# csteinmetz1/st-ito

Measured on AMD Instinct MI355X. Metric: candidate-evals/sec (pop x iters), 48 kHz 10 s stereo, 5-effect chain, higher is better.
Workload: dtype f32 (effects f32 / f64 as the reference; trunk convs with >= 256 output channels: f32 operands carried as f16 hi + lo pairs on the f16 matrix pipe, f32 accumulate -- as close to float64 as the f32 pipe, tools/ubench/split_mfma.hip)

## Files before the change

### st-ito_amd/csrc/compressor.hip

```cpp
#include "common.h"
#include "dsp_view.h"
#include "comp_scan.inc"

namespace stito {

static constexpr int CB_K = 15;
static constexpr int CB_TILE = 128;
static constexpr int CB_D = STITO_COMP_SCAN_DEPTH;
static constexpr int CA_TILE = 256;
static constexpr float CB_CMIN = 1.0e-30f;

typedef float cb_f2 __attribute__((ext_vector_type(2)));
typedef float cb_f4 __attribute__((ext_vector_type(4)));

struct CompGeom {
    int64_t L;
    int64_t n_blocks;
    int64_t n_fn;
    int64_t fn_stride;
    int64_t z_stride;
};

static CompGeom comp_geometry(int64_t L) {
    CompGeom g;
    g.L = L;
    g.n_blocks = (L + CB_K - 1) / CB_K;
    g.n_fn = g.n_blocks - 1;
    g.fn_stride = (g.n_fn + 2 * CB_D) * 16;
    g.z_stride = (g.n_fn + CB_D - 1) / CB_D * CB_D + CB_D;
    return g;
}

struct CompLayout : WsLayout { size_t fn, z_end; };
static CompLayout comp_layout(int n_streams, const CompGeom &g) {
    CompLayout l;
    l.fn = l.add((size_t)n_streams * g.fn_stride * sizeof(float));
    l.z_end = l.add((size_t)n_streams * g.z_stride * sizeof(float));
    return l;
}
size_t compressor_workspace_bytes(int n_streams, int64_t n_samples) { return comp_layout(n_streams, comp_geometry(n_samples)).total; }

struct CompCoef {
    float thr, thr_inv, p, cat, crl, sg;
};
__device__ __forceinline__ CompCoef comp_coef(const double *coef, int cand) {
    const double *cf = coef + (int64_t)cand * COEF_STRIDE;
    CompCoef c;
    c.thr = (float)cf[0];
    c.thr_inv = (float)cf[1];
    c.p = (float)cf[2];
    c.cat = (float)cf[3];
    c.crl = (float)cf[4];
    c.sg = c.cat <= c.crl ? 1.0f : -1.0f;
    return c;
}

template <int CTRL>
__device__ __forceinline__ float dpp(float old, float v) {
    return __builtin_bit_cast(float, __builtin_amdgcn_update_dpp(__builtin_bit_cast(int, old), __builtin_bit_cast(int, v),
                                                                 CTRL, 0xf, 0xf, false));
}

__global__ __launch_bounds__(256) void k_comp_blockfn(InView in, float *__restrict__ fn, CompGeom g, int C,
                                                       const double *__restrict__ coef) {
    __shared__ cb_f2 pairs[CB_TILE * CB_K];
    const int s = blockIdx.y, cand = s / C, ch = s % C;
    const float *x = in_ptr(in, cand, ch);
    const CompCoef cc = comp_coef(coef, cand);
    const float sa = cc.sg * (1.0f - cc.cat), sr = cc.sg * (1.0f - cc.crl);
    const cb_f2 c2 = {fmaxf(cc.cat, CB_CMIN), fmaxf(cc.crl, CB_CMIN)};
    const int64_t blk0 = (int64_t)blockIdx.x * CB_TILE, t0 = blk0 * CB_K;
    for (int i = threadIdx.x; i < CB_TILE * CB_K; i += 256) {
        const float v = t0 + i < g.L ? fabsf(x[t0 + i]) : 0.0f;
        pairs[i] = (cb_f2){sa * v, sr * v};
    }
    __syncthreads();
    const int lane = threadIdx.x & 63, w = threadIdx.x >> 6, row = lane >> 4, j = lane & 15;
    const float ninf = -__builtin_inff();
    float *out = fn + (int64_t)s * g.fn_stride;
#pragma unroll 2
    for (int it = 0; it < CB_TILE / 16; ++it) {
        const int bl = w * (CB_TILE / 4) + it * 4 + row;
        const cb_f2 *pr = pairs + bl * CB_K;
        float B = j == 0 ? 0.0f : ninf;
#pragma unroll
        for (int n = 0; n < CB_K; ++n) {
            const float sh = dpp<0x111>(ninf, B);
            const cb_f2 t = __builtin_elementwise_fma(c2, (cb_f2){sh, B}, pr[n]);
            B = fmaxf(t.x, t.y);
        }
        if (blk0 + bl < g.n_fn) out[(blk0 + bl) * 16 + j] = B;
    }
}

__global__ __launch_bounds__(64) void k_comp_blockscan(const float *__restrict__ fn, float *__restrict__ z_end, CompGeom g,
                                                        int C, int S, const double *__restrict__ coef, int spw) {
    const int lane = threadIdx.x, q = lane & 3;
    const int s_raw = blockIdx.x * spw + ((lane >> 2) & (spw - 1));
    const int s = s_raw < S ? s_raw : S - 1;
    const CompCoef cc = comp_coef(coef, s / C);
    const double ca = fmaxf(cc.cat, CB_CMIN), cr = fmaxf(cc.crl, CB_CMIN);
    float S4[4];
#pragma unroll
    for (int u = 0; u < 4; ++u) {
        const int jj = 4 * q + u;
        S4[u] = (float)(pow(ca, (double)jj) * pow(cr, (double)(CB_K - jj)));
    }
    const cb_f2 S01 = {S4[0], S4[1]}, S23 = {S4[2], S4[3]};
    const cb_f4 *src = (const cb_f4 *)(fn + (int64_t)s * g.fn_stride) + q;
    float *dst = z_end + (int64_t)s * g.z_stride;
    const int64_t n_ring = (g.n_fn + CB_D - 1) / CB_D;
    STITO_COMP_SCAN_PROLOGUE(src, dst + n_ring * CB_D);
    float z = 0.0f;
    for (int64_t r = 0; r < n_ring; ++r) {
        STITO_COMP_SCAN_PASS(z, S01, S23, src, dst);
        src += 4 * CB_D;
        dst += CB_D;
    }
    STITO_COMP_SCAN_DRAIN();
}

__device__ __forceinline__ float vca_gain(float e, float thr, float thr_inv, float p) {
    return e < thr ? 1.0f : __builtin_amdgcn_exp2f(p * __builtin_amdgcn_logf(e * thr_inv));
}

__global__ __launch_bounds__(CA_TILE) void k_comp_apply(InView in, float *out, const float *__restrict__ z_end,
                                                         CompGeom g, int64_t cand_stride, int C,
                                                         const double *__restrict__ coef) {
    __shared__ float tile[CA_TILE * CB_K];
    const int s = blockIdx.y, cand = s / C, ch = s % C;
    const float *x = in_ptr(in, cand, ch);
    float *y = out + (int64_t)cand * cand_stride + (int64_t)ch * g.L;
    const CompCoef cc = comp_coef(coef, cand);
    const int64_t blk0 = (int64_t)blockIdx.x * CA_TILE, t0 = blk0 * CB_K;
    const int n_here = (int)((g.L - t0 < CA_TILE * CB_K) ? g.L - t0 : CA_TILE * CB_K);
    for (int i = threadIdx.x; i < n_here; i += CA_TILE) tile[i] = x[t0 + i];
    const int64_t k = blk0 + threadIdx.x;
    float env = (k > 0 && k < g.n_blocks) ? fabsf(z_end[(int64_t)s * g.z_stride + k - 1]) : 0.0f;
    __syncthreads();
    float *mine = tile + threadIdx.x * CB_K;
    if (threadIdx.x * CB_K < n_here) {
#pragma unroll
        for (int n = 0; n < CB_K; ++n) {
            const float xv = mine[n], v = fabsf(xv);
            const float c = v > env ? cc.cat : cc.crl;
            env = __fadd_rn(v, __fmul_rn(c, __fsub_rn(env, v)));
            mine[n] = vca_gain(env, cc.thr, cc.thr_inv, cc.p) * xv;
        }
    }
    __syncthreads();
    for (int i = threadIdx.x; i < n_here; i += CA_TILE) y[t0 + i] = tile[i];
}

int compressor_stage(const InView &in, float *audio_dev, int64_t cand_stride, int pop, int C, int64_t n_samples,
                     const double *coef, void *workspace, hipStream_t st) {
    const CompGeom g = comp_geometry(n_samples);
    const int S = pop * C;
    const CompLayout l = comp_layout(S, g);
    float *fn = (float *)((char *)workspace + l.fn), *z_end = (float *)((char *)workspace + l.z_end);
    if (g.n_fn > 0) {
        hipLaunchKernelGGL(k_comp_blockfn, dim3((unsigned)((g.n_fn + CB_TILE - 1) / CB_TILE), S), dim3(256), 0, st, in, fn, g, C, coef);
        STITO_LAUNCH_CHECK();
        DeviceInfo dinfo;
        STITO_TRY(device_info(dinfo));
        int spw = 8;
        while (spw > 1 && (S + spw - 1) / spw < dinfo.cus / 4) spw >>= 1;
        if (const char *e = getenv("STITO_COMP_SPW")) { const int v = atoi(e); if (v >= 1 && v <= 16 && (v & (v - 1)) == 0) spw = v; }
        hipLaunchKernelGGL(k_comp_blockscan, dim3((S + spw - 1) / spw), dim3(64), 0, st, fn, z_end, g, C, S, coef, spw);
        STITO_LAUNCH_CHECK();
    }
    hipLaunchKernelGGL(k_comp_apply, dim3((unsigned)((g.n_blocks + CA_TILE - 1) / CA_TILE), S), dim3(CA_TILE), 0, st, in, audio_dev,
                       z_end, g, cand_stride, C, coef);
    STITO_LAUNCH_CHECK();
    return STITO_OK;
}

}
```

Measured before the change: 6048.

## Fuse compressor blockfn, scan and apply into one warp-specialized persistent kernel

Adds a single fused kernel per stream (or stream pair) in which producer waves compute block max-plus functions into LDS, one wave runs the serial scan in hand-written assembly, and consumer waves apply the gain and write output. The segments are pipelined across steps with double/triple-buffered LDS and barriers. This removes the global round-trips of the fn and z_end workspaces and two kernel launches. In exchange, parallelism is limited to one workgroup per stream or stream pair, and the code relies on hard-coded registers in inline asm. It becomes the default path and can be disabled with an environment variable.

Measured after the change: 6169 (median of 6 runs). 2.0% higher.

```diff
diff --git a/st-ito_amd/csrc/comp_stage.inc b/st-ito_amd/csrc/comp_stage.inc
--- /dev/null
+++ b/st-ito_amd/csrc/comp_stage.inc
@@ -0,0 +1,774 @@
+#define STITO_COMP_STAGE_G 64
+#define STITO_COMP_STAGE_SEGMENT(z, s01, s23, fn_lds, z_lds) \
+    asm volatile( \
+        "ds_write_b32 %4, %0 offset:12\n\t" \
+        "ds_read_b128 v[40:43], %3 offset:0\n\t" \
+        "ds_read_b128 v[44:47], %3 offset:64\n\t" \
+        "ds_read_b128 v[48:51], %3 offset:128\n\t" \
+        "ds_read_b128 v[52:55], %3 offset:192\n\t" \
+        "ds_read_b128 v[56:59], %3 offset:256\n\t" \
+        "ds_read_b128 v[60:63], %3 offset:320\n\t" \
+        "ds_read_b128 v[64:67], %3 offset:384\n\t" \
+        "ds_read_b128 v[68:71], %3 offset:448\n\t" \
+        "s_waitcnt lgkmcnt(4)\n\t" \
+        "v_mov_b32 v84, %0\n\t" \
+        "v_pk_fma_f32 v[80:81], %1, v[84:85], v[40:41] op_sel_hi:[1,0,1]\n\t" \
+        "v_pk_fma_f32 v[82:83], %2, v[84:85], v[42:43] op_sel_hi:[1,0,1]\n\t" \
+        "v_max_f32 v84, v80, v81\n\t" \
+        "v_max3_f32 v84, v84, v82, v83\n\t" \
+        "ds_read_b128 v[40:43], %3 offset:512\n\t" \
+        "s_nop 0\n\t" \
+        "v_max_f32_dpp v85, v84, v84 quad_perm:[1,0,3,2] row_mask:0xf bank_mask:0xf\n\t" \
+        "s_nop 1\n\t" \
+        "v_max_f32_dpp v72, v85, v85 quad_perm:[2,3,0,1] row_mask:0xf bank_mask:0xf\n\t" \
+        "v_pk_fma_f32 v[80:81], %1, v[72:73], v[44:45] op_sel_hi:[1,0,1]\n\t" \
+        "v_pk_fma_f32 v[82:83], %2, v[72:73], v[46:47] op_sel_hi:[1,0,1]\n\t" \
+        "v_max_f32 v84, v80, v81\n\t" \
+        "v_max3_f32 v84, v84, v82, v83\n\t" \
+        "ds_read_b128 v[44:47], %3 offset:576\n\t" \
+        "s_nop 0\n\t" \
+        "v_max_f32_dpp v85, v84, v84 quad_perm:[1,0,3,2] row_mask:0xf bank_mask:0xf\n\t" \
+        "s_nop 1\n\t" \
+        "v_max_f32_dpp v73, v85, v85 quad_perm:[2,3,0,1] row_mask:0xf bank_mask:0xf\n\t" \
+        "v_pk_fma_f32 v[80:81], %1, v[72:73], v[48:49] op_sel:[0,1,0] op_sel_hi:[1,1,1]\n\t" \
+        "v_pk_fma_f32 v[82:83], %2, v[72:73], v[50:51] op_sel:[0,1,0] op_sel_hi:[1,1,1]\n\t" \
+        "v_max_f32 v84, v80, v81\n\t" \
+        "v_max3_f32 v84, v84, v82, v83\n\t" \
+        "ds_read_b128 v[48:51], %3 offset:640\n\t" \
+        "s_nop 0\n\t" \
+        "v_max_f32_dpp v85, v84, v84 quad_perm:[1,0,3,2] row_mask:0xf bank_mask:0xf\n\t" \
+        "s_nop 1\n\t" \
+        "v_max_f32_dpp v74, v85, v85 quad_perm:[2,3,0,1] row_mask:0xf bank_mask:0xf\n\t" \
+        "v_pk_fma_f32 v[80:81], %1, v[74:75], v[52:53] op_sel_hi:[1,0,1]\n\t" \
+        "v_pk_fma_f32 v[82:83], %2, v[74:75], v[54:55] op_sel_hi:[1,0,1]\n\t" \
+        "v_max_f32 v84, v80, v81\n\t" \
+        "v_max3_f32 v84, v84, v82, v83\n\t" \
+        "ds_read_b128 v[52:55], %3 offset:704\n\t" \
+        "s_nop 0\n\t" \
+        "v_max_f32_dpp v85, v84, v84 quad_perm:[1,0,3,2] row_mask:0xf bank_mask:0xf\n\t" \
+        "s_nop 1\n\t" \
+        "v_max_f32_dpp v75, v85, v85 quad_perm:[2,3,0,1] row_mask:0xf bank_mask:0xf\n\t" \
+        "s_waitcnt lgkmcnt(4)\n\t" \
+        "v_pk_fma_f32 v[80:81], %1, v[74:75], v[56:57] op_sel:[0,1,0] op_sel_hi:[1,1,1]\n\t" \
+        "v_pk_fma_f32 v[82:83], %2, v[74:75], v[58:59] op_sel:[0,1,0] op_sel_hi:[1,1,1]\n\t" \
+        "v_max_f32 v84, v80, v81\n\t" \
+        "v_max3_f32 v84, v84, v82, v83\n\t" \
+        "ds_read_b128 v[56:59], %3 offset:768\n\t" \
+        "s_nop 0\n\t" \
+        "v_max_f32_dpp v85, v84, v84 quad_perm:[1,0,3,2] row_mask:0xf bank_mask:0xf\n\t" \
+        "s_nop 1\n\t" \
+        "v_max_f32_dpp v76, v85, v85 quad_perm:[2,3,0,1] row_mask:0xf bank_mask:0xf\n\t" \
+        "v_pk_fma_f32 v[80:81], %1, v[76:77], v[60:61] op_sel_hi:[1,0,1]\n\t" \
+        "v_pk_fma_f32 v[82:83], %2, v[76:77], v[62:63] op_sel_hi:[1,0,1]\n\t" \
+        "v_max_f32 v84, v80, v81\n\t" \
+        "v_max3_f32 v84, v84, v82, v83\n\t" \
+        "ds_read_b128 v[60:63], %3 offset:832\n\t" \
+        "s_nop 0\n\t" \
+        "v_max_f32_dpp v85, v84, v84 quad_perm:[1,0,3,2] row_mask:0xf bank_mask:0xf\n\t" \
+        "s_nop 1\n\t" \
+        "v_max_f32_dpp v77, v85, v85 quad_perm:[2,3,0,1] row_mask:0xf bank_mask:0xf\n\t" \
+        "v_pk_fma_f32 v[80:81], %1, v[76:77], v[64:65] op_sel:[0,1,0] op_sel_hi:[1,1,1]\n\t" \
+        "v_pk_fma_f32 v[82:83], %2, v[76:77], v[66:67] op_sel:[0,1,0] op_sel_hi:[1,1,1]\n\t" \
+        "v_max_f32 v84, v80, v81\n\t" \
+        "v_max3_f32 v84, v84, v82, v83\n\t" \
+        "ds_read_b128 v[64:67], %3 offset:896\n\t" \
+        "s_nop 0\n\t" \
+        "v_max_f32_dpp v85, v84, v84 quad_perm:[1,0,3,2] row_mask:0xf bank_mask:0xf\n\t" \
+        "s_nop 1\n\t" \
+        "v_max_f32_dpp v78, v85, v85 quad_perm:[2,3,0,1] row_mask:0xf bank_mask:0xf\n\t" \
+        "v_pk_fma_f32 v[80:81], %1, v[78:79], v[68:69] op_sel_hi:[1,0,1]\n\t" \
+        "v_pk_fma_f32 v[82:83], %2, v[78:79], v[70:71] op_sel_hi:[1,0,1]\n\t" \
+        "v_max_f32 v84, v80, v81\n\t" \
+        "v_max3_f32 v84, v84, v82, v83\n\t" \
+        "ds_read_b128 v[68:71], %3 offset:960\n\t" \
+        "s_nop 0\n\t" \
+        "v_max_f32_dpp v85, v84, v84 quad_perm:[1,0,3,2] row_mask:0xf bank_mask:0xf\n\t" \
+        "ds_write_b128 %4, v[72:75] offset:16\n\t" \
+        "s_nop 0\n\t" \
+        "v_max_f32_dpp v79, v85, v85 quad_perm:[2,3,0,1] row_mask:0xf bank_mask:0xf\n\t" \
+        "s_waitcnt lgkmcnt(5)\n\t" \
+        "v_pk_fma_f32 v[80:81], %1, v[78:79], v[40:41] op_sel:[0,1,0] op_sel_hi:[1,1,1]\n\t" \
+        "v_pk_fma_f32 v[82:83], %2, v[78:79], v[42:43] op_sel:[0,1,0] op_sel_hi:[1,1,1]\n\t" \
+        "v_max_f32 v84, v80, v81\n\t" \
+        "v_max3_f32 v84, v84, v82, v83\n\t" \
+        "ds_read_b128 v[40:43], %3 offset:1024\n\t" \
+        "s_nop 0\n\t" \
+        "v_max_f32_dpp v85, v84, v84 quad_perm:[1,0,3,2] row_mask:0xf bank_mask:0xf\n\t" \
+        "s_nop 1\n\t" \
+        "v_max_f32_dpp v72, v85, v85 quad_perm:[2,3,0,1] row_mask:0xf bank_mask:0xf\n\t" \
+        "v_pk_fma_f32 v[80:81], %1, v[72:73], v[44:45] op_sel_hi:[1,0,1]\n\t" \
+        "v_pk_fma_f32 v[82:83], %2, v[72:73], v[46:47] op_sel_hi:[1,0,1]\n\t" \
+        "v_max_f32 v84, v80, v81\n\t" \
+        "v_max3_f32 v84, v84, v82, v83\n\t" \
+        "ds_read_b128 v[44:47], %3 offset:1088\n\t" \
+        "s_nop 0\n\t" \
+        "v_max_f32_dpp v85, v84, v84 quad_perm:[1,0,3,2] row_mask:0xf bank_mask:0xf\n\t" \
+        "s_nop 1\n\t" \
+        "v_max_f32_dpp v73, v85, v85 quad_perm:[2,3,0,1] row_mask:0xf bank_mask:0xf\n\t" \
+        "v_pk_fma_f32 v[80:81], %1, v[72:73], v[48:49] op_sel:[0,1,0] op_sel_hi:[1,1,1]\n\t" \
+        "v_pk_fma_f32 v[82:83], %2, v[72:73], v[50:51] op_sel:[0,1,0] op_sel_hi:[1,1,1]\n\t" \
+        "v_max_f32 v84, v80, v81\n\t" \
+        "v_max3_f32 v84, v84, v82, v83\n\t" \
+        "ds_read_b128 v[48:51], %3 offset:1152\n\t" \
+        "s_nop 0\n\t" \
+        "v_max_f32_dpp v85, v84, v84 quad_perm:[1,0,3,2] row_mask:0xf bank_mask:0xf\n\t" \
+        "s_nop 1\n\t" \
+        "v_max_f32_dpp v74, v85, v85 quad_perm:[2,3,0,1] row_mask:0xf bank_mask:0xf\n\t" \
+        "v_pk_fma_f32 v[80:81], %1, v[74:75], v[52:53] op_sel_hi:[1,0,1]\n\t" \
+        "v_pk_fma_f32 v[82:83], %2, v[74:75], v[54:55] op_sel_hi:[1,0,1]\n\t" \
+        "v_max_f32 v84, v80, v81\n\t" \
+        "v_max3_f32 v84, v84, v82, v83\n\t" \
+        "ds_read_b128 v[52:55], %3 offset:1216\n\t" \
+        "s_nop 0\n\t" \
+        "v_max_f32_dpp v85, v84, v84 quad_perm:[1,0,3,2] row_mask:0xf bank_mask:0xf\n\t" \
+        "ds_write_b128 %4, v[76:79] offset:32\n\t" \
+        "s_nop 0\n\t" \
+        "v_max_f32_dpp v75, v85, v85 quad_perm:[2,3,0,1] row_mask:0xf bank_mask:0xf\n\t" \
+        "s_waitcnt lgkmcnt(6)\n\t" \
+        "v_pk_fma_f32 v[80:81], %1, v[74:75], v[56:57] op_sel:[0,1,0] op_sel_hi:[1,1,1]\n\t" \
+        "v_pk_fma_f32 v[82:83], %2, v[74:75], v[58:59] op_sel:[0,1,0] op_sel_hi:[1,1,1]\n\t" \
+        "v_max_f32 v84, v80, v81\n\t" \
+        "v_max3_f32 v84, v84, v82, v83\n\t" \
+        "ds_read_b128 v[56:59], %3 offset:1280\n\t" \
+        "s_nop 0\n\t" \
+        "v_max_f32_dpp v85, v84, v84 quad_perm:[1,0,3,2] row_mask:0xf bank_mask:0xf\n\t" \
+        "s_nop 1\n\t" \
+        "v_max_f32_dpp v76, v85, v85 quad_perm:[2,3,0,1] row_mask:0xf bank_mask:0xf\n\t" \
+        "v_pk_fma_f32 v[80:81], %1, v[76:77], v[60:61] op_sel_hi:[1,0,1]\n\t" \
+        "v_pk_fma_f32 v[82:83], %2, v[76:77], v[62:63] op_sel_hi:[1,0,1]\n\t" \
+        "v_max_f32 v84, v80, v81\n\t" \
+        "v_max3_f32 v84, v84, v82, v83\n\t" \
+        "ds_read_b128 v[60:63], %3 offset:1344\n\t" \
+        "s_nop 0\n\t" \
+        "v_max_f32_dpp v85, v84, v84 quad_perm:[1,0,3,2] row_mask:0xf bank_mask:0xf\n\t" \
+        "s_nop 1\n\t" \
+        "v_max_f32_dpp v77, v85, v85 quad_perm:[2,3,0,1] row_mask:0xf bank_mask:0xf\n\t" \
+        "v_pk_fma_f32 v[80:81], %1, v[76:77], v[64:65] op_sel:[0,1,0] op_sel_hi:[1,1,1]\n\t" \
+        "v_pk_fma_f32 v[82:83], %2, v[76:77], v[66:67] op_sel:[0,1,0] op_sel_hi:[1,1,1]\n\t" \
+        "v_max_f32 v84, v80, v81\n\t" \
+        "v_max3_f32 v84, v84, v82, v83\n\t" \
+        "ds_read_b128 v[64:67], %3 offset:1408\n\t" \
+        "s_nop 0\n\t" \
+        "v_max_f32_dpp v85, v84, v84 quad_perm:[1,0,3,2] row_mask:0xf bank_mask:0xf\n\t" \
+        "s_nop 1\n\t" \
+        "v_max_f32_dpp v78, v85, v85 quad_perm:[2,3,0,1] row_mask:0xf bank_mask:0xf\n\t" \
+        "v_pk_fma_f32 v[80:81], %1, v[78:79], v[68:69] op_sel_hi:[1,0,1]\n\t" \
+        "v_pk_fma_f32 v[82:83], %2, v[78:79], v[70:71] op_sel_hi:[1,0,1]\n\t" \
+        "v_max_f32 v84, v80, v81\n\t" \
+        "v_max3_f32 v84, v84, v82, v83\n\t" \
+        "ds_read_b128 v[68:71], %3 offset:1472\n\t" \
+        "s_nop 0\n\t" \
+        "v_max_f32_dpp v85, v84, v84 quad_perm:[1,0,3,2] row_mask:0xf bank_mask:0xf\n\t" \
+        "ds_write_b128 %4, v[72:75] offset:48\n\t" \
+        "s_nop 0\n\t" \
+        "v_max_f32_dpp v79, v85, v85 quad_perm:[2,3,0,1] row_mask:0xf bank_mask:0xf\n\t" \
+        "s_waitcnt lgkmcnt(6)\n\t" \
+        "v_pk_fma_f32 v[80:81], %1, v[78:79], v[40:41] op_sel:[0,1,0] op_sel_hi:[1,1,1]\n\t" \
+        "v_pk_fma_f32 v[82:83], %2, v[78:79], v[42:43] op_sel:[0,1,0] op_sel_hi:[1,1,1]\n\t" \
+        "v_max_f32 v84, v80, v81\n\t" \
+        "v_max3_f32 v84, v84, v82, v83\n\t" \
+        "ds_read_b128 v[40:43], %3 offset:1536\n\t" \
+        "s_nop 0\n\t" \
+        "v_max_f32_dpp v85, v84, v84 quad_perm:[1,0,3,2] row_mask:0xf bank_mask:0xf\n\t" \
+        "s_nop 1\n\t" \
+        "v_max_f32_dpp v72, v85, v85 quad_perm:[2,3,0,1] row_mask:0xf bank_mask:0xf\n\t" \
+        "v_pk_fma_f32 v[80:81], %1, v[72:73], v[44:45] op_sel_hi:[1,0,1]\n\t" \
+        "v_pk_fma_f32 v[82:83], %2, v[72:73], v[46:47] op_sel_hi:[1,0,1]\n\t" \
+        "v_max_f32 v84, v80, v81\n\t" \
+        "v_max3_f32 v84, v84, v82, v83\n\t" \
+        "ds_read_b128 v[44:47], %3 offset:1600\n\t" \
+        "s_nop 0\n\t" \
+        "v_max_f32_dpp v85, v84, v84 quad_perm:[1,0,3,2] row_mask:0xf bank_mask:0xf\n\t" \
+        "s_nop 1\n\t" \
+        "v_max_f32_dpp v73, v85, v85 quad_perm:[2,3,0,1] row_mask:0xf bank_mask:0xf\n\t" \
+        "v_pk_fma_f32 v[80:81], %1, v[72:73], v[48:49] op_sel:[0,1,0] op_sel_hi:[1,1,1]\n\t" \
+        "v_pk_fma_f32 v[82:83], %2, v[72:73], v[50:51] op_sel:[0,1,0] op_sel_hi:[1,1,1]\n\t" \
+        "v_max_f32 v84, v80, v81\n\t" \
+        "v_max3_f32 v84, v84, v82, v83\n\t" \
+        "ds_read_b128 v[48:51], %3 offset:1664\n\t" \
+        "s_nop 0\n\t" \
+        "v_max_f32_dpp v85, v84, v84 quad_perm:[1,0,3,2] row_mask:0xf bank_mask:0xf\n\t" \
+        "s_nop 1\n\t" \
+        "v_max_f32_dpp v74, v85, v85 quad_perm:[2,3,0,1] row_mask:0xf bank_mask:0xf\n\t" \
+        "v_pk_fma_f32 v[80:81], %1, v[74:75], v[52:53] op_sel_hi:[1,0,1]\n\t" \
+        "v_pk_fma_f32 v[82:83], %2, v[74:75], v[54:55] op_sel_hi:[1,0,1]\n\t" \
+        "v_max_f32 v84, v80, v81\n\t" \
+        "v_max3_f32 v84, v84, v82, v83\n\t" \
+        "ds_read_b128 v[52:55], %3 offset:1728\n\t" \
+        "s_nop 0\n\t" \
+        "v_max_f32_dpp v85, v84, v84 quad_perm:[1,0,3,2] row_mask:0xf bank_mask:0xf\n\t" \
+        "ds_write_b128 %4, v[76:79] offset:64\n\t" \
+        "s_nop 0\n\t" \
+        "v_max_f32_dpp v75, v85, v85 quad_perm:[2,3,0,1] row_mask:0xf bank_mask:0xf\n\t" \
+        "s_waitcnt lgkmcnt(6)\n\t" \
+        "v_pk_fma_f32 v[80:81], %1, v[74:75], v[56:57] op_sel:[0,1,0] op_sel_hi:[1,1,1]\n\t" \
+        "v_pk_fma_f32 v[82:83], %2, v[74:75], v[58:59] op_sel:[0,1,0] op_sel_hi:[1,1,1]\n\t" \
+        "v_max_f32 v84, v80, v81\n\t" \
+        "v_max3_f32 v84, v84, v82, v83\n\t" \
+        "ds_read_b128 v[56:59], %3 offset:1792\n\t" \
+        "s_nop 0\n\t" \
+        "v_max_f32_dpp v85, v84, v84 quad_perm:[1,0,3,2] row_mask:0xf bank_mask:0xf\n\t" \
+        "s_nop 1\n\t" \
+        "v_max_f32_dpp v76, v85, v85 quad_perm:[2,3,0,1] row_mask:0xf bank_mask:0xf\n\t" \
+        "v_pk_fma_f32 v[80:81], %1, v[76:77], v[60:61] op_sel_hi:[1,0,1]\n\t" \
+        "v_pk_fma_f32 v[82:83], %2, v[76:77], v[62:63] op_sel_hi:[1,0,1]\n\t" \
+        "v_max_f32 v84, v80, v81\n\t" \
+        "v_max3_f32 v84, v84, v82, v83\n\t" \
+        "ds_read_b128 v[60:63], %3 offset:1856\n\t" \
+        "s_nop 0\n\t" \
+        "v_max_f32_dpp v85, v84, v84 quad_perm:[1,0,3,2] row_mask:0xf bank_mask:0xf\n\t" \
+        "s_nop 1\n\t" \
+        "v_max_f32_dpp v77, v85, v85 quad_perm:[2,3,0,1] row_mask:0xf bank_mask:0xf\n\t" \
+        "v_pk_fma_f32 v[80:81], %1, v[76:77], v[64:65] op_sel:[0,1,0] op_sel_hi:[1,1,1]\n\t" \
+        "v_pk_fma_f32 v[82:83], %2, v[76:77], v[66:67] op_sel:[0,1,0] op_sel_hi:[1,1,1]\n\t" \
+        "v_max_f32 v84, v80, v81\n\t" \
+        "v_max3_f32 v84, v84, v82, v83\n\t" \
+        "ds_read_b128 v[64:67], %3 offset:1920\n\t" \
+        "s_nop 0\n\t" \
+        "v_max_f32_dpp v85, v84, v84 quad_perm:[1,0,3,2] row_mask:0xf bank_mask:0xf\n\t" \
+        "s_nop 1\n\t" \
+        "v_max_f32_dpp v78, v85, v85 quad_perm:[2,3,0,1] row_mask:0xf bank_mask:0xf\n\t" \
+        "v_pk_fma_f32 v[80:81], %1, v[78:79], v[68:69] op_sel_hi:[1,0,1]\n\t" \
+        "v_pk_fma_f32 v[82:83], %2, v[78:79], v[70:71] op_sel_hi:[1,0,1]\n\t" \
+        "v_max_f32 v84, v80, v81\n\t" \
+        "v_max3_f32 v84, v84, v82, v83\n\t" \
+        "ds_read_b128 v[68:71], %3 offset:1984\n\t" \
+        "s_nop 0\n\t" \
+        "v_max_f32_dpp v85, v84, v84 quad_perm:[1,0,3,2] row_mask:0xf bank_mask:0xf\n\t" \
+        "ds_write_b128 %4, v[72:75] offset:80\n\t" \
+        "s_nop 0\n\t" \
+        "v_max_f32_dpp v79, v85, v85 quad_perm:[2,3,0,1] row_mask:0xf bank_mask:0xf\n\t" \
+        "s_waitcnt lgkmcnt(6)\n\t" \
+        "v_pk_fma_f32 v[80:81], %1, v[78:79], v[40:41] op_sel:[0,1,0] op_sel_hi:[1,1,1]\n\t" \
+        "v_pk_fma_f32 v[82:83], %2, v[78:79], v[42:43] op_sel:[0,1,0] op_sel_hi:[1,1,1]\n\t" \
+        "v_max_f32 v84, v80, v81\n\t" \
+        "v_max3_f32 v84, v84, v82, v83\n\t" \
+        "ds_read_b128 v[40:43], %3 offset:2048\n\t" \
+        "s_nop 0\n\t" \
+        "v_max_f32_dpp v85, v84, v84 quad_perm:[1,0,3,2] row_mask:0xf bank_mask:0xf\n\t" \
+        "s_nop 1\n\t" \
+        "v_max_f32_dpp v72, v85, v85 quad_perm:[2,3,0,1] row_mask:0xf bank_mask:0xf\n\t" \
+        "v_pk_fma_f32 v[80:81], %1, v[72:73], v[44:45] op_sel_hi:[1,0,1]\n\t" \
+        "v_pk_fma_f32 v[82:83], %2, v[72:73], v[46:47] op_sel_hi:[1,0,1]\n\t" \
+        "v_max_f32 v84, v80, v81\n\t" \
+        "v_max3_f32 v84, v84, v82, v83\n\t" \
+        "ds_read_b128 v[44:47], %3 offset:2112\n\t" \
+        "s_nop 0\n\t" \
+        "v_max_f32_dpp v85, v84, v84 quad_perm:[1,0,3,2] row_mask:0xf bank_mask:0xf\n\t" \
+        "s_nop 1\n\t" \
+        "v_max_f32_dpp v73, v85, v85 quad_perm:[2,3,0,1] row_mask:0xf bank_mask:0xf\n\t" \
+        "v_pk_fma_f32 v[80:81], %1, v[72:73], v[48:49] op_sel:[0,1,0] op_sel_hi:[1,1,1]\n\t" \
+        "v_pk_fma_f32 v[82:83], %2, v[72:73], v[50:51] op_sel:[0,1,0] op_sel_hi:[1,1,1]\n\t" \
+        "v_max_f32 v84, v80, v81\n\t" \
+        "v_max3_f32 v84, v84, v82, v83\n\t" \
+        "ds_read_b128 v[48:51], %3 offset:2176\n\t" \
+        "s_nop 0\n\t" \
+        "v_max_f32_dpp v85, v84, v84 quad_perm:[1,0,3,2] row_mask:0xf bank_mask:0xf\n\t" \
+        "s_nop 1\n\t" \
+        "v_max_f32_dpp v74, v85, v85 quad_perm:[2,3,0,1] row_mask:0xf bank_mask:0xf\n\t" \
+        "v_pk_fma_f32 v[80:81], %1, v[74:75], v[52:53] op_sel_hi:[1,0,1]\n\t" \
+        "v_pk_fma_f32 v[82:83], %2, v[74:75], v[54:55] op_sel_hi:[1,0,1]\n\t" \
+        "v_max_f32 v84, v80, v81\n\t" \
+        "v_max3_f32 v84, v84, v82, v83\n\t" \
+        "ds_read_b128 v[52:55], %3 offset:2240\n\t" \
+        "s_nop 0\n\t" \
+        "v_max_f32_dpp v85, v84, v84 quad_perm:[1,0,3,2] row_mask:0xf bank_mask:0xf\n\t" \
+        "ds_write_b128 %4, v[76:79] offset:96\n\t" \
+        "s_nop 0\n\t" \
+        "v_max_f32_dpp v75, v85, v85 quad_perm:[2,3,0,1] row_mask:0xf bank_mask:0xf\n\t" \
+        "s_waitcnt lgkmcnt(6)\n\t" \
+        "v_pk_fma_f32 v[80:81], %1, v[74:75], v[56:57] op_sel:[0,1,0] op_sel_hi:[1,1,1]\n\t" \
+        "v_pk_fma_f32 v[82:83], %2, v[74:75], v[58:59] op_sel:[0,1,0] op_sel_hi:[1,1,1]\n\t" \
+        "v_max_f32 v84, v80, v81\n\t" \
+        "v_max3_f32 v84, v84, v82, v83\n\t" \
+        "ds_read_b128 v[56:59], %3 offset:2304\n\t" \
+        "s_nop 0\n\t" \
+        "v_max_f32_dpp v85, v84, v84 quad_perm:[1,0,3,2] row_mask:0xf bank_mask:0xf\n\t" \
+        "s_nop 1\n\t" \
+        "v_max_f32_dpp v76, v85, v85 quad_perm:[2,3,0,1] row_mask:0xf bank_mask:0xf\n\t" \
+        "v_pk_fma_f32 v[80:81], %1, v[76:77], v[60:61] op_sel_hi:[1,0,1]\n\t" \
+        "v_pk_fma_f32 v[82:83], %2, v[76:77], v[62:63] op_sel_hi:[1,0,1]\n\t" \
+        "v_max_f32 v84, v80, v81\n\t" \
+        "v_max3_f32 v84, v84, v82, v83\n\t" \
+        "ds_read_b128 v[60:63], %3 offset:2368\n\t" \
+        "s_nop 0\n\t" \
+        "v_max_f32_dpp v85, v84, v84 quad_perm:[1,0,3,2] row_mask:0xf bank_mask:0xf\n\t" \
+        "s_nop 1\n\t" \
+        "v_max_f32_dpp v77, v85, v85 quad_perm:[2,3,0,1] row_mask:0xf bank_mask:0xf\n\t" \
+        "v_pk_fma_f32 v[80:81], %1, v[76:77], v[64:65] op_sel:[0,1,0] op_sel_hi:[1,1,1]\n\t" \
+        "v_pk_fma_f32 v[82:83], %2, v[76:77], v[66:67] op_sel:[0,1,0] op_sel_hi:[1,1,1]\n\t" \
+        "v_max_f32 v84, v80, v81\n\t" \
+        "v_max3_f32 v84, v84, v82, v83\n\t" \
+        "ds_read_b128 v[64:67], %3 offset:2432\n\t" \
+        "s_nop 0\n\t" \
+        "v_max_f32_dpp v85, v84, v84 quad_perm:[1,0,3,2] row_mask:0xf bank_mask:0xf\n\t" \
+        "s_nop 1\n\t" \
+        "v_max_f32_dpp v78, v85, v85 quad_perm:[2,3,0,1] row_mask:0xf bank_mask:0xf\n\t" \
+        "v_pk_fma_f32 v[80:81], %1, v[78:79], v[68:69] op_sel_hi:[1,0,1]\n\t" \
+        "v_pk_fma_f32 v[82:83], %2, v[78:79], v[70:71] op_sel_hi:[1,0,1]\n\t" \
+        "v_max_f32 v84, v80, v81\n\t" \
+        "v_max3_f32 v84, v84, v82, v83\n\t" \
+        "ds_read_b128 v[68:71], %3 offset:2496\n\t" \
+        "s_nop 0\n\t" \
+        "v_max_f32_dpp v85, v84, v84 quad_perm:[1,0,3,2] row_mask:0xf bank_mask:0xf\n\t" \
+        "ds_write_b128 %4, v[72:75] offset:112\n\t" \
+        "s_nop 0\n\t" \
+        "v_max_f32_dpp v79, v85, v85 quad_perm:[2,3,0,1] row_mask:0xf bank_mask:0xf\n\t" \
+        "s_waitcnt lgkmcnt(6)\n\t" \
+        "v_pk_fma_f32 v[80:81], %1, v[78:79], v[40:41] op_sel:[0,1,0] op_sel_hi:[1,1,1]\n\t" \
+        "v_pk_fma_f32 v[82:83], %2, v[78:79], v[42:43] op_sel:[0,1,0] op_sel_hi:[1,1,1]\n\t" \
+        "v_max_f32 v84, v80, v81\n\t" \
+        "v_max3_f32 v84, v84, v82, v83\n\t" \
+        "ds_read_b128 v[40:43], %3 offset:2560\n\t" \
+        "s_nop 0\n\t" \
+        "v_max_f32_dpp v85, v84, v84 quad_perm:[1,0,3,2] row_mask:0xf bank_mask:0xf\n\t" \
+        "s_nop 1\n\t" \
+        "v_max_f32_dpp v72, v85, v85 quad_perm:[2,3,0,1] row_mask:0xf bank_mask:0xf\n\t" \
+        "v_pk_fma_f32 v[80:81], %1, v[72:73], v[44:45] op_sel_hi:[1,0,1]\n\t" \
+        "v_pk_fma_f32 v[82:83], %2, v[72:73], v[46:47] op_sel_hi:[1,0,1]\n\t" \
+        "v_max_f32 v84, v80, v81\n\t" \
+        "v_max3_f32 v84, v84, v82, v83\n\t" \
+        "ds_read_b128 v[44:47], %3 offset:2624\n\t" \
+        "s_nop 0\n\t" \
+        "v_max_f32_dpp v85, v84, v84 quad_perm:[1,0,3,2] row_mask:0xf bank_mask:0xf\n\t" \
+        "s_nop 1\n\t" \
+        "v_max_f32_dpp v73, v85, v85 quad_perm:[2,3,0,1] row_mask:0xf bank_mask:0xf\n\t" \
+        "v_pk_fma_f32 v[80:81], %1, v[72:73], v[48:49] op_sel:[0,1,0] op_sel_hi:[1,1,1]\n\t" \
+        "v_pk_fma_f32 v[82:83], %2, v[72:73], v[50:51] op_sel:[0,1,0] op_sel_hi:[1,1,1]\n\t" \
+        "v_max_f32 v84, v80, v81\n\t" \
+        "v_max3_f32 v84, v84, v82, v83\n\t" \
+        "ds_read_b128 v[48:51], %3 offset:2688\n\t" \
+        "s_nop 0\n\t" \
+        "v_max_f32_dpp v85, v84, v84 quad_perm:[1,0,3,2] row_mask:0xf bank_mask:0xf\n\t" \
+        "s_nop 1\n\t" \
+        "v_max_f32_dpp v74, v85, v85 quad_perm:[2,3,0,1] row_mask:0xf bank_mask:0xf\n\t" \
+        "v_pk_fma_f32 v[80:81], %1, v[74:75], v[52:53] op_sel_hi:[1,0,1]\n\t" \
+        "v_pk_fma_f32 v[82:83], %2, v[74:75], v[54:55] op_sel_hi:[1,0,1]\n\t" \
+        "v_max_f32 v84, v80, v81\n\t" \
+        "v_max3_f32 v84, v84, v82, v83\n\t" \
+        "ds_read_b128 v[52:55], %3 offset:2752\n\t" \
+        "s_nop 0\n\t" \
+        "v_max_f32_dpp v85, v84, v84 quad_perm:[1,0,3,2] row_mask:0xf bank_mask:0xf\n\t" \
+        "ds_write_b128 %4, v[76:79] offset:128\n\t" \
+        "s_nop 0\n\t" \
+        "v_max_f32_dpp v75, v85, v85 quad_perm:[2,3,0,1] row_mask:0xf bank_mask:0xf\n\t" \
+        "s_waitcnt lgkmcnt(6)\n\t" \
+        "v_pk_fma_f32 v[80:81], %1, v[74:75], v[56:57] op_sel:[0,1,0] op_sel_hi:[1,1,1]\n\t" \
+        "v_pk_fma_f32 v[82:83], %2, v[74:75], v[58:59] op_sel:[0,1,0] op_sel_hi:[1,1,1]\n\t" \
+        "v_max_f32 v84, v80, v81\n\t" \
+        "v_max3_f32 v84, v84, v82, v83\n\t" \
+        "ds_read_b128 v[56:59], %3 offset:2816\n\t" \
+        "s_nop 0\n\t" \
+        "v_max_f32_dpp v85, v84, v84 quad_perm:[1,0,3,2] row_mask:0xf bank_mask:0xf\n\t" \
+        "s_nop 1\n\t" \
+        "v_max_f32_dpp v76, v85, v85 quad_perm:[2,3,0,1] row_mask:0xf bank_mask:0xf\n\t" \
+        "v_pk_fma_f32 v[80:81], %1, v[76:77], v[60:61] op_sel_hi:[1,0,1]\n\t" \
+        "v_pk_fma_f32 v[82:83], %2, v[76:77], v[62:63] op_sel_hi:[1,0,1]\n\t" \
+        "v_max_f32 v84, v80, v81\n\t" \
+        "v_max3_f32 v84, v84, v82, v83\n\t" \
+        "ds_read_b128 v[60:63], %3 offset:2880\n\t" \
+        "s_nop 0\n\t" \
+        "v_max_f32_dpp v85, v84, v84 quad_perm:[1,0,3,2] row_mask:0xf bank_mask:0xf\n\t" \
+        "s_nop 1\n\t" \
+        "v_max_f32_dpp v77, v85, v85 quad_perm:[2,3,0,1] row_mask:0xf bank_mask:0xf\n\t" \
+        "v_pk_fma_f32 v[80:81], %1, v[76:77], v[64:65] op_sel:[0,1,0] op_sel_hi:[1,1,1]\n\t" \
+        "v_pk_fma_f32 v[82:83], %2, v[76:77], v[66:67] op_sel:[0,1,0] op_sel_hi:[1,1,1]\n\t" \
+        "v_max_f32 v84, v80, v81\n\t" \
+        "v_max3_f32 v84, v84, v82, v83\n\t" \
+        "ds_read_b128 v[64:67], %3 offset:2944\n\t" \
+        "s_nop 0\n\t" \
+        "v_max_f32_dpp v85, v84, v84 quad_perm:[1,0,3,2] row_mask:0xf bank_mask:0xf\n\t" \
+        "s_nop 1\n\t" \
+        "v_max_f32_dpp v78, v85, v85 quad_perm:[2,3,0,1] row_mask:0xf bank_mask:0xf\n\t" \
+        "v_pk_fma_f32 v[80:81], %1, v[78:79], v[68:69] op_sel_hi:[1,0,1]\n\t" \
+        "v_pk_fma_f32 v[82:83], %2, v[78:79], v[70:71] op_sel_hi:[1,0,1]\n\t" \
+        "v_max_f32 v84, v80, v81\n\t" \
+        "v_max3_f32 v84, v84, v82, v83\n\t" \
+        "ds_read_b128 v[68:71], %3 offset:3008\n\t" \
+        "s_nop 0\n\t" \
+        "v_max_f32_dpp v85, v84, v84 quad_perm:[1,0,3,2] row_mask:0xf bank_mask:0xf\n\t" \
+        "ds_write_b128 %4, v[72:75] offset:144\n\t" \
+        "s_nop 0\n\t" \
+        "v_max_f32_dpp v79, v85, v85 quad_perm:[2,3,0,1] row_mask:0xf bank_mask:0xf\n\t" \
+        "s_waitcnt lgkmcnt(6)\n\t" \
+        "v_pk_fma_f32 v[80:81], %1, v[78:79], v[40:41] op_sel:[0,1,0] op_sel_hi:[1,1,1]\n\t" \
+        "v_pk_fma_f32 v[82:83], %2, v[78:79], v[42:43] op_sel:[0,1,0] op_sel_hi:[1,1,1]\n\t" \
+        "v_max_f32 v84, v80, v81\n\t" \
+        "v_max3_f32 v84, v84, v82, v83\n\t" \
+        "ds_read_b128 v[40:43], %3 offset:3072\n\t" \
+        "s_nop 0\n\t" \
+        "v_max_f32_dpp v85, v84, v84 quad_perm:[1,0,3,2] row_mask:0xf bank_mask:0xf\n\t" \
+        "s_nop 1\n\t" \
+        "v_max_f32_dpp v72, v85, v85 quad_perm:[2,3,0,1] row_mask:0xf bank_mask:0xf\n\t" \
+        "v_pk_fma_f32 v[80:81], %1, v[72:73], v[44:45] op_sel_hi:[1,0,1]\n\t" \
+        "v_pk_fma_f32 v[82:83], %2, v[72:73], v[46:47] op_sel_hi:[1,0,1]\n\t" \
+        "v_max_f32 v84, v80, v81\n\t" \
+        "v_max3_f32 v84, v84, v82, v83\n\t" \
+        "ds_read_b128 v[44:47], %3 offset:3136\n\t" \
+        "s_nop 0\n\t" \
+        "v_max_f32_dpp v85, v84, v84 quad_perm:[1,0,3,2] row_mask:0xf bank_mask:0xf\n\t" \
+        "s_nop 1\n\t" \
+        "v_max_f32_dpp v73, v85, v85 quad_perm:[2,3,0,1] row_mask:0xf bank_mask:0xf\n\t" \
+        "v_pk_fma_f32 v[80:81], %1, v[72:73], v[48:49] op_sel:[0,1,0] op_sel_hi:[1,1,1]\n\t" \
+        "v_pk_fma_f32 v[82:83], %2, v[72:73], v[50:51] op_sel:[0,1,0] op_sel_hi:[1,1,1]\n\t" \
+        "v_max_f32 v84, v80, v81\n\t" \
+        "v_max3_f32 v84, v84, v82, v83\n\t" \
+        "ds_read_b128 v[48:51], %3 offset:3200\n\t" \
+        "s_nop 0\n\t" \
+        "v_max_f32_dpp v85, v84, v84 quad_perm:[1,0,3,2] row_mask:0xf bank_mask:0xf\n\t" \
+        "s_nop 1\n\t" \
+        "v_max_f32_dpp v74, v85, v85 quad_perm:[2,3,0,1] row_mask:0xf bank_mask:0xf\n\t" \
+        "v_pk_fma_f32 v[80:81], %1, v[74:75], v[52:53] op_sel_hi:[1,0,1]\n\t" \
+        "v_pk_fma_f32 v[82:83], %2, v[74:75], v[54:55] op_sel_hi:[1,0,1]\n\t" \
+        "v_max_f32 v84, v80, v81\n\t" \
+        "v_max3_f32 v84, v84, v82, v83\n\t" \
+        "ds_read_b128 v[52:55], %3 offset:3264\n\t" \
+        "s_nop 0\n\t" \
+        "v_max_f32_dpp v85, v84, v84 quad_perm:[1,0,3,2] row_mask:0xf bank_mask:0xf\n\t" \
+        "ds_write_b128 %4, v[76:79] offset:160\n\t" \
+        "s_nop 0\n\t" \
+        "v_max_f32_dpp v75, v85, v85 quad_perm:[2,3,0,1] row_mask:0xf bank_mask:0xf\n\t" \
+        "s_waitcnt lgkmcnt(6)\n\t" \
+        "v_pk_fma_f32 v[80:81], %1, v[74:75], v[56:57] op_sel:[0,1,0] op_sel_hi:[1,1,1]\n\t" \
+        "v_pk_fma_f32 v[82:83], %2, v[74:75], v[58:59] op_sel:[0,1,0] op_sel_hi:[1,1,1]\n\t" \
+        "v_max_f32 v84, v80, v81\n\t" \
+        "v_max3_f32 v84, v84, v82, v83\n\t" \
+        "ds_read_b128 v[56:59], %3 offset:3328\n\t" \
+        "s_nop 0\n\t" \
+        "v_max_f32_dpp v85, v84, v84 quad_perm:[1,0,3,2] row_mask:0xf bank_mask:0xf\n\t" \
+        "s_nop 1\n\t" \
+        "v_max_f32_dpp v76, v85, v85 quad_perm:[2,3,0,1] row_mask:0xf bank_mask:0xf\n\t" \
+        "v_pk_fma_f32 v[80:81], %1, v[76:77], v[60:61] op_sel_hi:[1,0,1]\n\t" \
+        "v_pk_fma_f32 v[82:83], %2, v[76:77], v[62:63] op_sel_hi:[1,0,1]\n\t" \
+        "v_max_f32 v84, v80, v81\n\t" \
+        "v_max3_f32 v84, v84, v82, v83\n\t" \
+        "ds_read_b128 v[60:63], %3 offset:3392\n\t" \
+        "s_nop 0\n\t" \
+        "v_max_f32_dpp v85, v84, v84 quad_perm:[1,0,3,2] row_mask:0xf bank_mask:0xf\n\t" \
+        "s_nop 1\n\t" \
+        "v_max_f32_dpp v77, v85, v85 quad_perm:[2,3,0,1] row_mask:0xf bank_mask:0xf\n\t" \
+        "v_pk_fma_f32 v[80:81], %1, v[76:77], v[64:65] op_sel:[0,1,0] op_sel_hi:[1,1,1]\n\t" \
+        "v_pk_fma_f32 v[82:83], %2, v[76:77], v[66:67] op_sel:[0,1,0] op_sel_hi:[1,1,1]\n\t" \
+        "v_max_f32 v84, v80, v81\n\t" \
+        "v_max3_f32 v84, v84, v82, v83\n\t" \
+        "ds_read_b128 v[64:67], %3 offset:3456\n\t" \
+        "s_nop 0\n\t" \
+        "v_max_f32_dpp v85, v84, v84 quad_perm:[1,0,3,2] row_mask:0xf bank_mask:0xf\n\t" \
+        "s_nop 1\n\t" \
+        "v_max_f32_dpp v78, v85, v85 quad_perm:[2,3,0,1] row_mask:0xf bank_mask:0xf\n\t" \
+        "v_pk_fma_f32 v[80:81], %1, v[78:79], v[68:69] op_sel_hi:[1,0,1]\n\t" \
+        "v_pk_fma_f32 v[82:83], %2, v[78:79], v[70:71] op_sel_hi:[1,0,1]\n\t" \
+        "v_max_f32 v84, v80, v81\n\t" \
+        "v_max3_f32 v84, v84, v82, v83\n\t" \
+        "ds_read_b128 v[68:71], %3 offset:3520\n\t" \
+        "s_nop 0\n\t" \
+        "v_max_f32_dpp v85, v84, v84 quad_perm:[1,0,3,2] row_mask:0xf bank_mask:0xf\n\t" \
+        "ds_write_b128 %4, v[72:75] offset:176\n\t" \
+        "s_nop 0\n\t" \
+        "v_max_f32_dpp v79, v85, v85 quad_perm:[2,3,0,1] row_mask:0xf bank_mask:0xf\n\t" \
+        "s_waitcnt lgkmcnt(6)\n\t" \
+        "v_pk_fma_f32 v[80:81], %1, v[78:79], v[40:41] op_sel:[0,1,0] op_sel_hi:[1,1,1]\n\t" \
+        "v_pk_fma_f32 v[82:83], %2, v[78:79], v[42:43] op_sel:[0,1,0] op_sel_hi:[1,1,1]\n\t" \
+        "v_max_f32 v84, v80, v81\n\t" \
+        "v_max3_f32 v84, v84, v82, v83\n\t" \
+        "ds_read_b128 v[40:43], %3 offset:3584\n\t" \
+        "s_nop 0\n\t" \
+        "v_max_f32_dpp v85, v84, v84 quad_perm:[1,0,3,2] row_mask:0xf bank_mask:0xf\n\t" \
+        "s_nop 1\n\t" \
+        "v_max_f32_dpp v72, v85, v85 quad_perm:[2,3,0,1] row_mask:0xf bank_mask:0xf\n\t" \
+        "v_pk_fma_f32 v[80:81], %1, v[72:73], v[44:45] op_sel_hi:[1,0,1]\n\t" \
+        "v_pk_fma_f32 v[82:83], %2, v[72:73], v[46:47] op_sel_hi:[1,0,1]\n\t" \
+        "v_max_f32 v84, v80, v81\n\t" \
+        "v_max3_f32 v84, v84, v82, v83\n\t" \
+        "ds_read_b128 v[44:47], %3 offset:3648\n\t" \
+        "s_nop 0\n\t" \
+        "v_max_f32_dpp v85, v84, v84 quad_perm:[1,0,3,2] row_mask:0xf bank_mask:0xf\n\t" \
+        "s_nop 1\n\t" \
+        "v_max_f32_dpp v73, v85, v85 quad_perm:[2,3,0,1] row_mask:0xf bank_mask:0xf\n\t" \
+        "v_pk_fma_f32 v[80:81], %1, v[72:73], v[48:49] op_sel:[0,1,0] op_sel_hi:[1,1,1]\n\t" \
+        "v_pk_fma_f32 v[82:83], %2, v[72:73], v[50:51] op_sel:[0,1,0] op_sel_hi:[1,1,1]\n\t" \
+        "v_max_f32 v84, v80, v81\n\t" \
+        "v_max3_f32 v84, v84, v82, v83\n\t" \
+        "ds_read_b128 v[48:51], %3 offset:3712\n\t" \
+        "s_nop 0\n\t" \
+        "v_max_f32_dpp v85, v84, v84 quad_perm:[1,0,3,2] row_mask:0xf bank_mask:0xf\n\t" \
+        "s_nop 1\n\t" \
+        "v_max_f32_dpp v74, v85, v85 quad_perm:[2,3,0,1] row_mask:0xf bank_mask:0xf\n\t" \
+        "v_pk_fma_f32 v[80:81], %1, v[74:75], v[52:53] op_sel_hi:[1,0,1]\n\t" \
+        "v_pk_fma_f32 v[82:83], %2, v[74:75], v[54:55] op_sel_hi:[1,0,1]\n\t" \
+        "v_max_f32 v84, v80, v81\n\t" \
+        "v_max3_f32 v84, v84, v82, v83\n\t" \
+        "ds_read_b128 v[52:55], %3 offset:3776\n\t" \
+        "s_nop 0\n\t" \
+        "v_max_f32_dpp v85, v84, v84 quad_perm:[1,0,3,2] row_mask:0xf bank_mask:0xf\n\t" \
+        "ds_write_b128 %4, v[76:79] offset:192\n\t" \
+        "s_nop 0\n\t" \
+        "v_max_f32_dpp v75, v85, v85 quad_perm:[2,3,0,1] row_mask:0xf bank_mask:0xf\n\t" \
+        "s_waitcnt lgkmcnt(6)\n\t" \
+        "v_pk_fma_f32 v[80:81], %1, v[74:75], v[56:57] op_sel:[0,1,0] op_sel_hi:[1,1,1]\n\t" \
+        "v_pk_fma_f32 v[82:83], %2, v[74:75], v[58:59] op_sel:[0,1,0] op_sel_hi:[1,1,1]\n\t" \
+        "v_max_f32 v84, v80, v81\n\t" \
+        "v_max3_f32 v84, v84, v82, v83\n\t" \
+        "ds_read_b128 v[56:59], %3 offset:3840\n\t" \
+        "s_nop 0\n\t" \
+        "v_max_f32_dpp v85, v84, v84 quad_perm:[1,0,3,2] row_mask:0xf bank_mask:0xf\n\t" \
+        "s_nop 1\n\t" \
+        "v_max_f32_dpp v76, v85, v85 quad_perm:[2,3,0,1] row_mask:0xf bank_mask:0xf\n\t" \
+        "v_pk_fma_f32 v[80:81], %1, v[76:77], v[60:61] op_sel_hi:[1,0,1]\n\t" \
+        "v_pk_fma_f32 v[82:83], %2, v[76:77], v[62:63] op_sel_hi:[1,0,1]\n\t" \
+        "v_max_f32 v84, v80, v81\n\t" \
+        "v_max3_f32 v84, v84, v82, v83\n\t" \
+        "ds_read_b128 v[60:63], %3 offset:3904\n\t" \
+        "s_nop 0\n\t" \
+        "v_max_f32_dpp v85, v84, v84 quad_perm:[1,0,3,2] row_mask:0xf bank_mask:0xf\n\t" \
+        "s_nop 1\n\t" \
+        "v_max_f32_dpp v77, v85, v85 quad_perm:[2,3,0,1] row_mask:0xf bank_mask:0xf\n\t" \
+        "v_pk_fma_f32 v[80:81], %1, v[76:77], v[64:65] op_sel:[0,1,0] op_sel_hi:[1,1,1]\n\t" \
+        "v_pk_fma_f32 v[82:83], %2, v[76:77], v[66:67] op_sel:[0,1,0] op_sel_hi:[1,1,1]\n\t" \
+        "v_max_f32 v84, v80, v81\n\t" \
+        "v_max3_f32 v84, v84, v82, v83\n\t" \
+        "ds_read_b128 v[64:67], %3 offset:3968\n\t" \
+        "s_nop 0\n\t" \
+        "v_max_f32_dpp v85, v84, v84 quad_perm:[1,0,3,2] row_mask:0xf bank_mask:0xf\n\t" \
+        "s_nop 1\n\t" \
+        "v_max_f32_dpp v78, v85, v85 quad_perm:[2,3,0,1] row_mask:0xf bank_mask:0xf\n\t" \
+        "v_pk_fma_f32 v[80:81], %1, v[78:79], v[68:69] op_sel_hi:[1,0,1]\n\t" \
+        "v_pk_fma_f32 v[82:83], %2, v[78:79], v[70:71] op_sel_hi:[1,0,1]\n\t" \
+        "v_max_f32 v84, v80, v81\n\t" \
+        "v_max3_f32 v84, v84, v82, v83\n\t" \
+        "ds_read_b128 v[68:71], %3 offset:4032\n\t" \
+        "s_nop 0\n\t" \
+        "v_max_f32_dpp v85, v84, v84 quad_perm:[1,0,3,2] row_mask:0xf bank_mask:0xf\n\t" \
+        "ds_write_b128 %4, v[72:75] offset:208\n\t" \
+        "s_nop 0\n\t" \
+        "v_max_f32_dpp v79, v85, v85 quad_perm:[2,3,0,1] row_mask:0xf bank_mask:0xf\n\t" \
+        "s_waitcnt lgkmcnt(6)\n\t" \
+        "v_pk_fma_f32 v[80:81], %1, v[78:79], v[40:41] op_sel:[0,1,0] op_sel_hi:[1,1,1]\n\t" \
+        "v_pk_fma_f32 v[82:83], %2, v[78:79], v[42:43] op_sel:[0,1,0] op_sel_hi:[1,1,1]\n\t" \
+        "v_max_f32 v84, v80, v81\n\t" \
+        "v_max3_f32 v84, v84, v82, v83\n\t" \
+        "s_nop 1\n\t" \
+        "v_max_f32_dpp v85, v84, v84 quad_perm:[1,0,3,2] row_mask:0xf bank_mask:0xf\n\t" \
+        "s_nop 1\n\t" \
+        "v_max_f32_dpp v72, v85, v85 quad_perm:[2,3,0,1] row_mask:0xf bank_mask:0xf\n\t" \
+        "v_pk_fma_f32 v[80:81], %1, v[72:73], v[44:45] op_sel_hi:[1,0,1]\n\t" \
+        "v_pk_fma_f32 v[82:83], %2, v[72:73], v[46:47] op_sel_hi:[1,0,1]\n\t" \
+        "v_max_f32 v84, v80, v81\n\t" \
+        "v_max3_f32 v84, v84, v82, v83\n\t" \
+        "s_nop 1\n\t" \
+        "v_max_f32_dpp v85, v84, v84 quad_perm:[1,0,3,2] row_mask:0xf bank_mask:0xf\n\t" \
+        "s_nop 1\n\t" \
+        "v_max_f32_dpp v73, v85, v85 quad_perm:[2,3,0,1] row_mask:0xf bank_mask:0xf\n\t" \
+        "v_pk_fma_f32 v[80:81], %1, v[72:73], v[48:49] op_sel:[0,1,0] op_sel_hi:[1,1,1]\n\t" \
+        "v_pk_fma_f32 v[82:83], %2, v[72:73], v[50:51] op_sel:[0,1,0] op_sel_hi:[1,1,1]\n\t" \
+        "v_max_f32 v84, v80, v81\n\t" \
+        "v_max3_f32 v84, v84, v82, v83\n\t" \
+        "s_nop 1\n\t" \
+        "v_max_f32_dpp v85, v84, v84 quad_perm:[1,0,3,2] row_mask:0xf bank_mask:0xf\n\t" \
+        "s_nop 1\n\t" \
+        "v_max_f32_dpp v74, v85, v85 quad_perm:[2,3,0,1] row_mask:0xf bank_mask:0xf\n\t" \
+        "v_pk_fma_f32 v[80:81], %1, v[74:75], v[52:53] op_sel_hi:[1,0,1]\n\t" \
+        "v_pk_fma_f32 v[82:83], %2, v[74:75], v[54:55] op_sel_hi:[1,0,1]\n\t" \
+        "v_max_f32 v84, v80, v81\n\t" \
+        "v_max3_f32 v84, v84, v82, v83\n\t" \
+        "s_nop 1\n\t" \
+        "v_max_f32_dpp v85, v84, v84 quad_perm:[1,0,3,2] row_mask:0xf bank_mask:0xf\n\t" \
+        "ds_write_b128 %4, v[76:79] offset:224\n\t" \
+        "s_nop 0\n\t" \
+        "v_max_f32_dpp v75, v85, v85 quad_perm:[2,3,0,1] row_mask:0xf bank_mask:0xf\n\t" \
+        "s_waitcnt lgkmcnt(2)\n\t" \
+        "v_pk_fma_f32 v[80:81], %1, v[74:75], v[56:57] op_sel:[0,1,0] op_sel_hi:[1,1,1]\n\t" \
+        "v_pk_fma_f32 v[82:83], %2, v[74:75], v[58:59] op_sel:[0,1,0] op_sel_hi:[1,1,1]\n\t" \
+        "v_max_f32 v84, v80, v81\n\t" \
+        "v_max3_f32 v84, v84, v82, v83\n\t" \
+        "s_nop 1\n\t" \
+        "v_max_f32_dpp v85, v84, v84 quad_perm:[1,0,3,2] row_mask:0xf bank_mask:0xf\n\t" \
+        "s_nop 1\n\t" \
+        "v_max_f32_dpp v76, v85, v85 quad_perm:[2,3,0,1] row_mask:0xf bank_mask:0xf\n\t" \
+        "v_pk_fma_f32 v[80:81], %1, v[76:77], v[60:61] op_sel_hi:[1,0,1]\n\t" \
+        "v_pk_fma_f32 v[82:83], %2, v[76:77], v[62:63] op_sel_hi:[1,0,1]\n\t" \
+        "v_max_f32 v84, v80, v81\n\t" \
+        "v_max3_f32 v84, v84, v82, v83\n\t" \
+        "s_nop 1\n\t" \
+        "v_max_f32_dpp v85, v84, v84 quad_perm:[1,0,3,2] row_mask:0xf bank_mask:0xf\n\t" \
+        "s_nop 1\n\t" \
+        "v_max_f32_dpp v77, v85, v85 quad_perm:[2,3,0,1] row_mask:0xf bank_mask:0xf\n\t" \
+        "v_pk_fma_f32 v[80:81], %1, v[76:77], v[64:65] op_sel:[0,1,0] op_sel_hi:[1,1,1]\n\t" \
+        "v_pk_fma_f32 v[82:83], %2, v[76:77], v[66:67] op_sel:[0,1,0] op_sel_hi:[1,1,1]\n\t" \
+        "v_max_f32 v84, v80, v81\n\t" \
+        "v_max3_f32 v84, v84, v82, v83\n\t" \
+        "s_nop 1\n\t" \
+        "v_max_f32_dpp v85, v84, v84 quad_perm:[1,0,3,2] row_mask:0xf bank_mask:0xf\n\t" \
+        "s_nop 1\n\t" \
+        "v_max_f32_dpp v78, v85, v85 quad_perm:[2,3,0,1] row_mask:0xf bank_mask:0xf\n\t" \
+        "v_pk_fma_f32 v[80:81], %1, v[78:79], v[68:69] op_sel_hi:[1,0,1]\n\t" \
+        "v_pk_fma_f32 v[82:83], %2, v[78:79], v[70:71] op_sel_hi:[1,0,1]\n\t" \
+        "v_max_f32 v84, v80, v81\n\t" \
+        "v_max3_f32 v84, v84, v82, v83\n\t" \
+        "s_nop 1\n\t" \
+        "v_max_f32_dpp v85, v84, v84 quad_perm:[1,0,3,2] row_mask:0xf bank_mask:0xf\n\t" \
+        "ds_write_b128 %4, v[72:75] offset:240\n\t" \
+        "s_nop 0\n\t" \
+        "v_max_f32_dpp v79, v85, v85 quad_perm:[2,3,0,1] row_mask:0xf bank_mask:0xf\n\t" \
+        "ds_write_b128 %4, v[76:79] offset:256\n\t" \
+        "v_mov_b32 %0, v79\n\t" \
+        "s_waitcnt lgkmcnt(0)\n\t" \
+        : "+v"(z) : "v"(s01), "v"(s23), "v"(fn_lds), "v"(z_lds) : "memory", "v40", "v41", "v42", "v43", "v44", "v45", "v46", "v47", "v48", "v49", "v50", "v51", "v52", "v53", "v54", "v55", "v56", "v57", "v58", "v59", "v60", "v61", "v62", "v63", "v64", "v65", "v66", "v67", "v68", "v69", "v70", "v71", "v72", "v73", "v74", "v75", "v76", "v77", "v78", "v79", "v80", "v81", "v82", "v83", "v84", "v85")
+#define STITO_COMP_STAGE_BLOCKFN2(b_a, b_b, c2, sa, sr, b_init, x_lds) \
+    asm volatile( \
+        "ds_read2_b32 v[40:41], %6 offset0:0 offset1:60\n\t" \
+        "ds_read2_b32 v[42:43], %6 offset0:1 offset1:61\n\t" \
+        "ds_read2_b32 v[44:45], %6 offset0:2 offset1:62\n\t" \
+        "ds_read2_b32 v[46:47], %6 offset0:3 offset1:63\n\t" \
+        "ds_read2_b32 v[48:49], %6 offset0:4 offset1:64\n\t" \
+        "ds_read2_b32 v[50:51], %6 offset0:5 offset1:65\n\t" \
+        "ds_read2_b32 v[52:53], %6 offset0:6 offset1:66\n\t" \
+        "ds_read2_b32 v[54:55], %6 offset0:7 offset1:67\n\t" \
+        "ds_read2_b32 v[56:57], %6 offset0:8 offset1:68\n\t" \
+        "ds_read2_b32 v[58:59], %6 offset0:9 offset1:69\n\t" \
+        "ds_read2_b32 v[60:61], %6 offset0:10 offset1:70\n\t" \
+        "ds_read2_b32 v[62:63], %6 offset0:11 offset1:71\n\t" \
+        "ds_read2_b32 v[64:65], %6 offset0:12 offset1:72\n\t" \
+        "ds_read2_b32 v[66:67], %6 offset0:13 offset1:73\n\t" \
+        "ds_read2_b32 v[68:69], %6 offset0:14 offset1:74\n\t" \
+        "v_mov_b32 v79, %5\n\t" \
+        "v_mov_b32 v81, %5\n\t" \
+        "s_waitcnt lgkmcnt(14)\n\t" \
+        "v_mul_f32_e64 v70, %3, |v40|\n\t" \
+        "v_mul_f32_e64 v71, %4, |v40|\n\t" \
+        "v_mul_f32_e64 v72, %3, |v41|\n\t" \
+        "v_mul_f32_e64 v73, %4, |v41|\n\t" \
+        "v_pk_fma_f32 v[78:79], %2, v[78:79], v[70:71] op_sel:[0,1,0] op_sel_hi:[1,1,1]\n\t" \
+        "v_pk_fma_f32 v[80:81], %2, v[80:81], v[72:73] op_sel:[0,1,0] op_sel_hi:[1,1,1]\n\t" \
+        "s_waitcnt lgkmcnt(13)\n\t" \
+        "v_mul_f32_e64 v74, %3, |v42|\n\t" \
+        "v_mul_f32_e64 v75, %4, |v42|\n\t" \
+        "v_max_f32_dpp v79, v78, v79 row_shr:1 row_mask:0xf bank_mask:0xf\n\t" \
+        "v_max_f32_dpp v81, v80, v81 row_shr:1 row_mask:0xf bank_mask:0xf\n\t" \
+        "v_mul_f32_e64 v76, %3, |v43|\n\t" \
+        "v_mul_f32_e64 v77, %4, |v43|\n\t" \
+        "v_pk_fma_f32 v[78:79], %2, v[78:79], v[74:75] op_sel:[0,1,0] op_sel_hi:[1,1,1]\n\t" \
+        "v_pk_fma_f32 v[80:81], %2, v[80:81], v[76:77] op_sel:[0,1,0] op_sel_hi:[1,1,1]\n\t" \
+        "s_waitcnt lgkmcnt(12)\n\t" \
+        "v_mul_f32_e64 v70, %3, |v44|\n\t" \
+        "v_mul_f32_e64 v71, %4, |v44|\n\t" \
+        "v_max_f32_dpp v79, v78, v79 row_shr:1 row_mask:0xf bank_mask:0xf\n\t" \
+        "v_max_f32_dpp v81, v80, v81 row_shr:1 row_mask:0xf bank_mask:0xf\n\t" \
+        "v_mul_f32_e64 v72, %3, |v45|\n\t" \
+        "v_mul_f32_e64 v73, %4, |v45|\n\t" \
+        "v_pk_fma_f32 v[78:79], %2, v[78:79], v[70:71] op_sel:[0,1,0] op_sel_hi:[1,1,1]\n\t" \
+        "v_pk_fma_f32 v[80:81], %2, v[80:81], v[72:73] op_sel:[0,1,0] op_sel_hi:[1,1,1]\n\t" \
+        "s_waitcnt lgkmcnt(11)\n\t" \
+        "v_mul_f32_e64 v74, %3, |v46|\n\t" \
+        "v_mul_f32_e64 v75, %4, |v46|\n\t" \
+        "v_max_f32_dpp v79, v78, v79 row_shr:1 row_mask:0xf bank_mask:0xf\n\t" \
+        "v_max_f32_dpp v81, v80, v81 row_shr:1 row_mask:0xf bank_mask:0xf\n\t" \
+        "v_mul_f32_e64 v76, %3, |v47|\n\t" \
+        "v_mul_f32_e64 v77, %4, |v47|\n\t" \
+        "v_pk_fma_f32 v[78:79], %2, v[78:79], v[74:75] op_sel:[0,1,0] op_sel_hi:[1,1,1]\n\t" \
+        "v_pk_fma_f32 v[80:81], %2, v[80:81], v[76:77] op_sel:[0,1,0] op_sel_hi:[1,1,1]\n\t" \
+        "s_waitcnt lgkmcnt(10)\n\t" \
+        "v_mul_f32_e64 v70, %3, |v48|\n\t" \
+        "v_mul_f32_e64 v71, %4, |v48|\n\t" \
+        "v_max_f32_dpp v79, v78, v79 row_shr:1 row_mask:0xf bank_mask:0xf\n\t" \
+        "v_max_f32_dpp v81, v80, v81 row_shr:1 row_mask:0xf bank_mask:0xf\n\t" \
+        "v_mul_f32_e64 v72, %3, |v49|\n\t" \
+        "v_mul_f32_e64 v73, %4, |v49|\n\t" \
+        "v_pk_fma_f32 v[78:79], %2, v[78:79], v[70:71] op_sel:[0,1,0] op_sel_hi:[1,1,1]\n\t" \
+        "v_pk_fma_f32 v[80:81], %2, v[80:81], v[72:73] op_sel:[0,1,0] op_sel_hi:[1,1,1]\n\t" \
+        "s_waitcnt lgkmcnt(9)\n\t" \
+        "v_mul_f32_e64 v74, %3, |v50|\n\t" \
+        "v_mul_f32_e64 v75, %4, |v50|\n\t" \
+        "v_max_f32_dpp v79, v78, v79 row_shr:1 row_mask:0xf bank_mask:0xf\n\t" \
+        "v_max_f32_dpp v81, v80, v81 row_shr:1 row_mask:0xf bank_mask:0xf\n\t" \
+        "v_mul_f32_e64 v76, %3, |v51|\n\t" \
+        "v_mul_f32_e64 v77, %4, |v51|\n\t" \
+        "v_pk_fma_f32 v[78:79], %2, v[78:79], v[74:75] op_sel:[0,1,0] op_sel_hi:[1,1,1]\n\t" \
+        "v_pk_fma_f32 v[80:81], %2, v[80:81], v[76:77] op_sel:[0,1,0] op_sel_hi:[1,1,1]\n\t" \
+        "s_waitcnt lgkmcnt(8)\n\t" \
+        "v_mul_f32_e64 v70, %3, |v52|\n\t" \
+        "v_mul_f32_e64 v71, %4, |v52|\n\t" \
+        "v_max_f32_dpp v79, v78, v79 row_shr:1 row_mask:0xf bank_mask:0xf\n\t" \
+        "v_max_f32_dpp v81, v80, v81 row_shr:1 row_mask:0xf bank_mask:0xf\n\t" \
+        "v_mul_f32_e64 v72, %3, |v53|\n\t" \
+        "v_mul_f32_e64 v73, %4, |v53|\n\t" \
+        "v_pk_fma_f32 v[78:79], %2, v[78:79], v[70:71] op_sel:[0,1,0] op_sel_hi:[1,1,1]\n\t" \
+        "v_pk_fma_f32 v[80:81], %2, v[80:81], v[72:73] op_sel:[0,1,0] op_sel_hi:[1,1,1]\n\t" \
+        "s_waitcnt lgkmcnt(7)\n\t" \
+        "v_mul_f32_e64 v74, %3, |v54|\n\t" \
+        "v_mul_f32_e64 v75, %4, |v54|\n\t" \
+        "v_max_f32_dpp v79, v78, v79 row_shr:1 row_mask:0xf bank_mask:0xf\n\t" \
+        "v_max_f32_dpp v81, v80, v81 row_shr:1 row_mask:0xf bank_mask:0xf\n\t" \
+        "v_mul_f32_e64 v76, %3, |v55|\n\t" \
+        "v_mul_f32_e64 v77, %4, |v55|\n\t" \
+        "v_pk_fma_f32 v[78:79], %2, v[78:79], v[74:75] op_sel:[0,1,0] op_sel_hi:[1,1,1]\n\t" \
+        "v_pk_fma_f32 v[80:81], %2, v[80:81], v[76:77] op_sel:[0,1,0] op_sel_hi:[1,1,1]\n\t" \
+        "s_waitcnt lgkmcnt(6)\n\t" \
+        "v_mul_f32_e64 v70, %3, |v56|\n\t" \
+        "v_mul_f32_e64 v71, %4, |v56|\n\t" \
+        "v_max_f32_dpp v79, v78, v79 row_shr:1 row_mask:0xf bank_mask:0xf\n\t" \
+        "v_max_f32_dpp v81, v80, v81 row_shr:1 row_mask:0xf bank_mask:0xf\n\t" \
+        "v_mul_f32_e64 v72, %3, |v57|\n\t" \
+        "v_mul_f32_e64 v73, %4, |v57|\n\t" \
+        "v_pk_fma_f32 v[78:79], %2, v[78:79], v[70:71] op_sel:[0,1,0] op_sel_hi:[1,1,1]\n\t" \
+        "v_pk_fma_f32 v[80:81], %2, v[80:81], v[72:73] op_sel:[0,1,0] op_sel_hi:[1,1,1]\n\t" \
+        "s_waitcnt lgkmcnt(5)\n\t" \
+        "v_mul_f32_e64 v74, %3, |v58|\n\t" \
+        "v_mul_f32_e64 v75, %4, |v58|\n\t" \
+        "v_max_f32_dpp v79, v78, v79 row_shr:1 row_mask:0xf bank_mask:0xf\n\t" \
+        "v_max_f32_dpp v81, v80, v81 row_shr:1 row_mask:0xf bank_mask:0xf\n\t" \
+        "v_mul_f32_e64 v76, %3, |v59|\n\t" \
+        "v_mul_f32_e64 v77, %4, |v59|\n\t" \
+        "v_pk_fma_f32 v[78:79], %2, v[78:79], v[74:75] op_sel:[0,1,0] op_sel_hi:[1,1,1]\n\t" \
+        "v_pk_fma_f32 v[80:81], %2, v[80:81], v[76:77] op_sel:[0,1,0] op_sel_hi:[1,1,1]\n\t" \
+        "s_waitcnt lgkmcnt(4)\n\t" \
+        "v_mul_f32_e64 v70, %3, |v60|\n\t" \
+        "v_mul_f32_e64 v71, %4, |v60|\n\t" \
+        "v_max_f32_dpp v79, v78, v79 row_shr:1 row_mask:0xf bank_mask:0xf\n\t" \
+        "v_max_f32_dpp v81, v80, v81 row_shr:1 row_mask:0xf bank_mask:0xf\n\t" \
+        "v_mul_f32_e64 v72, %3, |v61|\n\t" \
+        "v_mul_f32_e64 v73, %4, |v61|\n\t" \
+        "v_pk_fma_f32 v[78:79], %2, v[78:79], v[70:71] op_sel:[0,1,0] op_sel_hi:[1,1,1]\n\t" \
+        "v_pk_fma_f32 v[80:81], %2, v[80:81], v[72:73] op_sel:[0,1,0] op_sel_hi:[1,1,1]\n\t" \
+        "s_waitcnt lgkmcnt(3)\n\t" \
+        "v_mul_f32_e64 v74, %3, |v62|\n\t" \
+        "v_mul_f32_e64 v75, %4, |v62|\n\t" \
+        "v_max_f32_dpp v79, v78, v79 row_shr:1 row_mask:0xf bank_mask:0xf\n\t" \
+        "v_max_f32_dpp v81, v80, v81 row_shr:1 row_mask:0xf bank_mask:0xf\n\t" \
+        "v_mul_f32_e64 v76, %3, |v63|\n\t" \
+        "v_mul_f32_e64 v77, %4, |v63|\n\t" \
+        "v_pk_fma_f32 v[78:79], %2, v[78:79], v[74:75] op_sel:[0,1,0] op_sel_hi:[1,1,1]\n\t" \
+        "v_pk_fma_f32 v[80:81], %2, v[80:81], v[76:77] op_sel:[0,1,0] op_sel_hi:[1,1,1]\n\t" \
+        "s_waitcnt lgkmcnt(2)\n\t" \
+        "v_mul_f32_e64 v70, %3, |v64|\n\t" \
+        "v_mul_f32_e64 v71, %4, |v64|\n\t" \
+        "v_max_f32_dpp v79, v78, v79 row_shr:1 row_mask:0xf bank_mask:0xf\n\t" \
+        "v_max_f32_dpp v81, v80, v81 row_shr:1 row_mask:0xf bank_mask:0xf\n\t" \
+        "v_mul_f32_e64 v72, %3, |v65|\n\t" \
+        "v_mul_f32_e64 v73, %4, |v65|\n\t" \
+        "v_pk_fma_f32 v[78:79], %2, v[78:79], v[70:71] op_sel:[0,1,0] op_sel_hi:[1,1,1]\n\t" \
+        "v_pk_fma_f32 v[80:81], %2, v[80:81], v[72:73] op_sel:[0,1,0] op_sel_hi:[1,1,1]\n\t" \
+        "s_waitcnt lgkmcnt(1)\n\t" \
+        "v_mul_f32_e64 v74, %3, |v66|\n\t" \
+        "v_mul_f32_e64 v75, %4, |v66|\n\t" \
+        "v_max_f32_dpp v79, v78, v79 row_shr:1 row_mask:0xf bank_mask:0xf\n\t" \
+        "v_max_f32_dpp v81, v80, v81 row_shr:1 row_mask:0xf bank_mask:0xf\n\t" \
+        "v_mul_f32_e64 v76, %3, |v67|\n\t" \
+        "v_mul_f32_e64 v77, %4, |v67|\n\t" \
+        "v_pk_fma_f32 v[78:79], %2, v[78:79], v[74:75] op_sel:[0,1,0] op_sel_hi:[1,1,1]\n\t" \
+        "v_pk_fma_f32 v[80:81], %2, v[80:81], v[76:77] op_sel:[0,1,0] op_sel_hi:[1,1,1]\n\t" \
+        "s_waitcnt lgkmcnt(0)\n\t" \
+        "v_mul_f32_e64 v70, %3, |v68|\n\t" \
+        "v_mul_f32_e64 v71, %4, |v68|\n\t" \
+        "v_max_f32_dpp v79, v78, v79 row_shr:1 row_mask:0xf bank_mask:0xf\n\t" \
+        "v_max_f32_dpp v81, v80, v81 row_shr:1 row_mask:0xf bank_mask:0xf\n\t" \
+        "v_mul_f32_e64 v72, %3, |v69|\n\t" \
+        "v_mul_f32_e64 v73, %4, |v69|\n\t" \
+        "v_pk_fma_f32 v[78:79], %2, v[78:79], v[70:71] op_sel:[0,1,0] op_sel_hi:[1,1,1]\n\t" \
+        "v_pk_fma_f32 v[80:81], %2, v[80:81], v[72:73] op_sel:[0,1,0] op_sel_hi:[1,1,1]\n\t" \
+        "s_nop 1\n\t" \
+        "v_max_f32_dpp v79, v78, v79 row_shr:1 row_mask:0xf bank_mask:0xf\n\t" \
+        "v_max_f32_dpp v81, v80, v81 row_shr:1 row_mask:0xf bank_mask:0xf\n\t" \
+        "v_mov_b32 %0, v79\n\t" \
+        "v_mov_b32 %1, v81\n\t" \
+        : "=&v"(b_a), "=&v"(b_b) : "v"(c2), "v"(sa), "v"(sr), "v"(b_init), "v"(x_lds) : "memory", "v40", "v41", "v42", "v43", "v44", "v45", "v46", "v47", "v48", "v49", "v50", "v51", "v52", "v53", "v54", "v55", "v56", "v57", "v58", "v59", "v60", "v61", "v62", "v63", "v64", "v65", "v66", "v67", "v68", "v69", "v70", "v71", "v72", "v73", "v74", "v75", "v76", "v77", "v78", "v79", "v80", "v81")
diff --git a/st-ito_amd/csrc/compressor.hip b/st-ito_amd/csrc/compressor.hip
--- a/st-ito_amd/csrc/compressor.hip
+++ b/st-ito_amd/csrc/compressor.hip
@@ -1,6 +1,7 @@
 #include "common.h"
 #include "dsp_view.h"
 #include "comp_scan.inc"
+#include "comp_stage.inc"
 
 namespace stito {
 
@@ -152,17 +153,208 @@
     for (int i = threadIdx.x; i < n_here; i += CA_TILE) y[t0 + i] = tile[i];
 }
 
+static constexpr int CS_G = STITO_COMP_STAGE_G;
+static constexpr int CS_SEG = CS_G * CB_K;
+static constexpr int CS_NH = 12;
+static constexpr int CS_THREADS = 16 * 64;
+static constexpr int CS_UNIT = 4 * CB_K;
+static constexpr int CS_UPS = CS_G / 4;
+static constexpr int CS_ZS = 4 + CS_G;
+
+#define CS_BARRIER() asm volatile("s_waitcnt lgkmcnt(0)\n\ts_barrier" ::: "memory")
+#define CS_WAVE_SYNC() do { __builtin_amdgcn_fence(__ATOMIC_RELEASE, "wavefront"); __builtin_amdgcn_wave_barrier(); \
+                            __builtin_amdgcn_fence(__ATOMIC_ACQUIRE, "wavefront"); } while (0)
+
+__device__ __forceinline__ uint32_t cs_lds_addr(const void *p) {
+    return (uint32_t)(uintptr_t)(const __attribute__((address_space(3))) void *)p;
+}
+
+template <int NS> struct CsSplit;
+template <> struct CsSplit<1> { static constexpr int MAXU = 2; static constexpr int first[CS_NH] = {0, 4, 10, 2, 6, 12, 14, 8, 14, 14, 14, 14}, count[CS_NH] = {2, 2, 2, 2, 2, 2, 0, 2, 2, 0, 0, 0}, c_stream[CS_NH] = {-1, -1, -1, -1, -1, -1, -1, -1, -1, 0, -1, -1}; };
+template <> struct CsSplit<2> { static constexpr int MAXU = 4; static constexpr int first[CS_NH] = {0, 16, 10, 4, 20, 26, 8, 24, 14, 28, 28, 30}, count[CS_NH] = {4, 4, 4, 4, 4, 4, 2, 2, 2, 0, 0, 2}, c_stream[CS_NH] = {-1, -1, -1, -1, -1, -1, -1, -1, -1, 0, 1, -1}; };
+
+template <int NS> struct CsLds {
+    static constexpr int fn = 0;
+    static constexpr int z = fn + 2 * NS * CS_G * 16;
+    static constexpr int cf = z + 2 * NS * CS_ZS;
+    static constexpr int x = cf + NS * 4;
+    static constexpr int total = x + 3 * NS * CS_SEG;
+    static_assert(z % 4 == 0 && cf % 4 == 0, "b128 alignment");
+    static_assert(total * 4 <= 64 * 1024, "beyond this a launch has to raise hipFuncAttributeMaxDynamicSharedMemorySize first");
+};
+
+template <int NS>
+__global__ __launch_bounds__(CS_THREADS) void k_comp_stage(InView in, float *out, CompGeom g, int64_t cand_stride, int C, int S,
+                                                     const double *__restrict__ coef) {
+    typedef CsSplit<NS> SP;
+    typedef CsLds<NS> LD;
+    extern __shared__ __attribute__((aligned(16))) float cs_smem[];
+    float (*s_fn)[NS][CS_G * 16] = (float (*)[NS][CS_G * 16])(cs_smem + LD::fn);
+    float (*s_z)[NS][CS_ZS] = (float (*)[NS][CS_ZS])(cs_smem + LD::z);
+    float (*s_cf)[4] = (float (*)[4])(cs_smem + LD::cf);
+    float (*s_x)[NS][CS_SEG] = (float (*)[NS][CS_SEG])(cs_smem + LD::x);
+    const int lane = threadIdx.x & 63, w = threadIdx.x >> 6;
+    const int s0 = blockIdx.x * NS;
+    const int n_seg = (int)((g.n_blocks + CS_G - 1) / CS_G), n_steps = (n_seg + 2 + 2) / 3 * 3;
+    if (threadIdx.x < NS) {
+        const int s = s0 + threadIdx.x < S ? s0 + threadIdx.x : S - 1;
+        const CompCoef cc = comp_coef(coef, s / C);
+        s_cf[threadIdx.x][0] = cc.sg * (1.0f - cc.cat);
+        s_cf[threadIdx.x][1] = cc.sg * (1.0f - cc.crl);
+        s_cf[threadIdx.x][2] = fmaxf(cc.cat, CB_CMIN);
+        s_cf[threadIdx.x][3] = fmaxf(cc.crl, CB_CMIN);
+    }
+    CS_BARRIER();
+    if (w == 0) {
+        const int q = lane & 3, sl = (lane >> 2) % NS;
+        const int s = s0 + sl < S ? s0 + sl : S - 1;
+        const CompCoef cc = comp_coef(coef, s / C);
+        const double ca = fmaxf(cc.cat, CB_CMIN), cr = fmaxf(cc.crl, CB_CMIN);
+        float S4[4];
+#pragma unroll
+        for (int u = 0; u < 4; ++u) {
+            const int jj = 4 * q + u;
+            S4[u] = (float)(pow(ca, (double)jj) * pow(cr, (double)(CB_K - jj)));
+        }
+        const cb_f2 S01 = {S4[0], S4[1]}, S23 = {S4[2], S4[3]};
+        const uint32_t fn0 = cs_lds_addr(&s_fn[0][sl][4 * q]), fn1 = cs_lds_addr(&s_fn[1][sl][4 * q]);
+        const uint32_t z0 = cs_lds_addr(&s_z[0][sl][0]), z1 = cs_lds_addr(&s_z[1][sl][0]);
+        float z = 0.0f;
+        if (lane < 4 * NS) {
+            for (int t = 0; t < n_steps; ++t) {
+                if (t >= 1 && t <= n_seg) {
+                    const uint32_t fa = (t - 1) & 1 ? fn1 : fn0, za = (t - 1) & 1 ? z1 : z0;
+                    STITO_COMP_STAGE_SEGMENT(z, S01, S23, fa, za);
+                }
+                CS_BARRIER();
+            }
+        }
+    } else if ((w & 3) == 0) {
+        for (int t = 0; t < n_steps; ++t) CS_BARRIER();
+    } else {
+        const int h = w - 1 - (w >> 2), u0 = SP::first[h], un = SP::count[h], c_sl = SP::c_stream[h];
+        if (c_sl >= 0) {
+            const int c_s = s0 + c_sl;
+            const bool c_on = c_s < S;
+            const int c_sc = c_on ? c_s : S - 1;
+            const CompCoef cc = comp_coef(coef, c_sc / C);
+            float *y = out + (int64_t)(c_sc / C) * cand_stride + (int64_t)(c_sc % C) * g.L;
+            float cat = cc.cat, crl = cc.crl;
+            asm volatile("" : "+v"(cat), "+v"(crl));
+            for (int t = 0; t < n_steps; ++t) {
+                if (c_on && t >= 2 && t - 2 < n_seg) {
+                    const int seg = t - 2;
+                    float *xb = &s_x[seg % 3][c_sl][0];
+                    float env = fabsf(s_z[seg & 1][c_sl][3 + lane]);
+                    float *mine = xb + lane * CB_K;
+                    float xv[CB_K];
+#pragma unroll
+                    for (int n = 0; n < CB_K; ++n) xv[n] = mine[n];
+#pragma unroll
+                    for (int n = 0; n < CB_K; ++n) {
+                        const float v = fabsf(xv[n]);
+                        const float c = v > env ? cat : crl;
+                        env = __fadd_rn(v, __fmul_rn(c, __fsub_rn(env, v)));
+                        xv[n] = vca_gain(env, cc.thr, cc.thr_inv, cc.p) * xv[n];
+                    }
+#pragma unroll
+                    for (int n = 0; n < CB_K; ++n) mine[n] = xv[n];
+                    CS_WAVE_SYNC();
+                    const int64_t t0 = (int64_t)seg * CS_SEG;
+                    const int64_t left = g.L - t0;
+                    const int n_here = (int)(left < CS_SEG ? left : CS_SEG);
+                    float *yb = y + t0;
+#pragma unroll
+                    for (int n = 0; n < CB_K; ++n) xv[n] = xb[n * 64 + lane];
+                    if (n_here == CS_SEG) {
+#pragma unroll
+                        for (int n = 0; n < CB_K; ++n) yb[n * 64 + lane] = xv[n];
+                    } else {
+#pragma unroll
+                        for (int n = 0; n < CB_K; ++n) {
+                            const int i = n * 64 + lane;
+                            if (i < n_here) yb[i] = xv[n];
+                        }
+                    }
+                }
+                CS_BARRIER();
+            }
+        } else {
+            const int row = lane >> 4, j = lane & 15;
+            const float ninf = -__builtin_inff();
+            const int a_sl = u0 / CS_UPS < NS ? u0 / CS_UPS : NS - 1;
+            const int a_s = s0 + a_sl < S ? s0 + a_sl : S - 1;
+            const float *xa = in_ptr(in, a_s / C, a_s % C);
+            const cb_f4 cf = *(const cb_f4 *)s_cf[a_sl];
+            const cb_f2 c2 = {cf.z, cf.w};
+            const int off0 = (u0 % CS_UPS) * CS_UNIT + lane;
+
+            float r0[SP::MAXU], r1[SP::MAXU], r2[SP::MAXU];
+            auto fetch = [&](float (&dst)[SP::MAXU], int seg) {
+                const int segc = seg < n_seg ? seg : n_seg - 1;
+                const int64_t left = g.L - (int64_t)segc * CS_SEG;
+                const int last = (int)(left < CS_SEG ? left : CS_SEG) - 1;
+                const float *xb = xa + (int64_t)segc * CS_SEG;
+#pragma unroll
+                for (int i = 0; i < SP::MAXU; ++i) {
+                    const int o = off0 + i * CS_UNIT;
+                    dst[i] = xb[o < last ? o : last];
+                }
+            };
+            fetch(r0, 0);
+            fetch(r1, 1);
+            auto step = [&](int t, const float (&cur)[SP::MAXU], float (&ahead)[SP::MAXU]) {
+                fetch(ahead, t + 2);
+                const int64_t left_t = g.L - (int64_t)t * CS_SEG;
+                const int n_t = (int)(left_t < 0 ? 0 : left_t < CS_SEG ? left_t : CS_SEG);
+                float *xs = &s_x[t % 3][0][0] + u0 * CS_UNIT;
+                float *fo = &s_fn[t & 1][0][0] + u0 * 64 + lane;
+#pragma unroll
+                for (int i = 0; i < SP::MAXU; ++i)
+                    if (i < un && lane < CS_UNIT) xs[i * CS_UNIT + lane] = off0 + i * CS_UNIT < n_t ? cur[i] : 0.0f;
+                CS_WAVE_SYNC();
+                const uint32_t x_row = cs_lds_addr(xs + row * CB_K);
+#pragma unroll 1
+                for (int i = 0; i < un; i += 2) {
+                    float Ba, Bb;
+                    STITO_COMP_STAGE_BLOCKFN2(Ba, Bb, c2, cf.x, cf.y, j == 0 ? 0.0f : ninf, x_row + i * (CS_UNIT * 4));
+                    fo[i * 64] = Ba;
+                    if (i + 1 < un) fo[(i + 1) * 64] = Bb;
+                }
+                CS_BARRIER();
+            };
+            for (int t = 0; t < n_steps; t += 3) {
+                step(t, r0, r2);
+                step(t + 1, r1, r0);
+                step(t + 2, r2, r1);
+            }
+        }
+    }
+}
+
 int compressor_stage(const InView &in, float *audio_dev, int64_t cand_stride, int pop, int C, int64_t n_samples,
                      const double *coef, void *workspace, hipStream_t st) {
     const CompGeom g = comp_geometry(n_samples);
     const int S = pop * C;
+    DeviceInfo dinfo;
+    STITO_TRY(device_info(dinfo));
+    const char *fused = getenv("STITO_COMP_FUSED");
+    if (!(fused && atoi(fused) == 0)) {
+        int ns = S > dinfo.cus ? 2 : 1;
+        if (const char *e = getenv("STITO_COMP_NS")) { const int v = atoi(e); if (v == 1 || v == 2) ns = v; }
+        if (ns == 2) {
+            hipLaunchKernelGGL(k_comp_stage<2>, dim3((S + 1) / 2), dim3(CS_THREADS), CsLds<2>::total * 4, st, in, audio_dev, g, cand_stride, C, S, coef);
+        } else {
+            hipLaunchKernelGGL(k_comp_stage<1>, dim3(S), dim3(CS_THREADS), CsLds<1>::total * 4, st, in, audio_dev, g, cand_stride, C, S, coef);
+        }
+        STITO_LAUNCH_CHECK();
+        return STITO_OK;
+    }
     const CompLayout l = comp_layout(S, g);
     float *fn = (float *)((char *)workspace + l.fn), *z_end = (float *)((char *)workspace + l.z_end);
     if (g.n_fn > 0) {
         hipLaunchKernelGGL(k_comp_blockfn, dim3((unsigned)((g.n_fn + CB_TILE - 1) / CB_TILE), S), dim3(256), 0, st, in, fn, g, C, coef);
         STITO_LAUNCH_CHECK();
-        DeviceInfo dinfo;
-        STITO_TRY(device_info(dinfo));
         int spw = 8;
         while (spw > 1 && (S + spw - 1) / spw < dinfo.cus / 4) spw >>= 1;
         if (const char *e = getenv("STITO_COMP_SPW")) { const int v = atoi(e); if (v >= 1 && v <= 16 && (v & (v - 1)) == 0) spw = v; }
```
